# polarsignals/frostdb

Hardware: AMD Instinct MI355X
Metric: rows/sec filter+group-by on 1B-row Prometheus Arrow (HBM-resident); achieved HBM GB/s vs peak (higher is better)
Workload: dtype f64; 1 GPU; headline: Prometheus schema, labels.code=='200' + SUM(value) GROUP BY labels.path; total_rows=1000000000, rows_per_gpu=1000000000, records_per_gpu=40, groups=1025, parallelism=1 GPU

## Files before the change

### frostdb_amd/csrc/fdb_capi.cpp

```cpp
#include <cstring>
#include <new>
#include <string>
#include <vector>

#include "fdb_codec.h"
#include "fdb_comm.h"
#include "fdb_context.h"
#include "fdb_dynamic.h"
#include "fdb_jit.h"
#include "fdb_mergepath.h"
#include "fdb_mergerec.h"
#include "fdb_plan.h"
#include "fdb_pqwrite_host.h"
#include "fdb_record.h"
#include "fdb_regex.h"
#include "fdb_sort.h"
#include "fdb_sortkey.h"
#include "fdb_take.h"

struct fdb_plan {
  std::unique_ptr<fdb::DynamicAggs> dyn;
  fdb_plan_desc main_desc;
  fdb::Plan plan;
  fdb_plan(const fdb_plan_desc* d, int dev)
// ... 106 lines not shown
      fdb::widen_indices_mapped(src, width + 10, table, width == -12 ? 4 : 16, dst, (size_t)n);
      return;
    }
    fdb::widen_indices(src, width, dst, (size_t)n);
  });
}

int fdb_selftest_scan_cache(const uint32_t* indices, int64_t rows, int32_t width, int device, uint8_t* out, int64_t out_bytes) {
  return guard(nullptr, [&] {
    if (indices == nullptr || out == nullptr || rows <= 0 || rows > ((int64_t)1 << 28) || (width != 1 && width != 2) || out_bytes != (rows * width + 15) / 16 * 16)
      throw fdb::Error(FDB_ERR_INVALID, "scan cache: 1 to 2^28 rows, width 1 or 2, out_bytes = rows * width rounded up to 16");
    fdb::CallScope call(device);
    void* d_src = call.alloc(fdb::values_slot((size_t)rows, 4));
    void* d_dst = call.alloc(fdb::values_slot((size_t)rows, (size_t)width));
    fdb::hip_check(hipMemcpyAsync(d_src, indices, (size_t)rows * 4, hipMemcpyHostToDevice, call.ctx->stream), "scan cache: copy in");
    fdb::hip_check(fdb_launch_narrow_indices((const uint32_t*)d_src, d_dst, rows, width, call.ctx->stream), "scan cache: builder");
    fdb::hip_check(hipMemcpyAsync(out, d_dst, (size_t)out_bytes, hipMemcpyDeviceToHost, call.ctx->stream), "scan cache: copy out");
    fdb::hip_check(hipStreamSynchronize(call.ctx->stream), "scan cache: wait");
    for (int64_t i = 0; i < rows; i++) {
      const int64_t at = fdb::scan_cache_position(i, rows, width);
      const uint32_t got = width == 1 ? out[at] : (uint32_t)out[2 * at] | ((uint32_t)out[2 * at + 1] << 8);
      if (got != (indices[i] & (width == 1 ? 0xFFu : 0xFFFFu))) throw fdb::Error(FDB_ERR_INVALID, "scan cache: row " + std::to_string(i) + " is not at its position");
    }
  });
}

int fdb_selftest_exact_sum(const double* x, int64_t n, double* out) {
  return guard(nullptr, [&] {
    if (n < 0 || out == nullptr || (n > 0 && x == nullptr)) throw fdb::Error(FDB_ERR_INVALID, "exact sum: n >= 0 and non-null buffers");
    long long limbs[FDB_EXACT_LIMBS] = {0};
    unsigned long long flags = 0;
    int64_t since = 0;
    for (int64_t i = 0; i < n; i++) {
      unsigned long long bits;
      std::memcpy(&bits, x + i, 8);
      int k; long long d0, d1, d2;
      const unsigned long long f = fdb_exact_split(bits, &k, &d0, &d1, &d2);
      if (f != 0ull) { flags |= f; continue; }
      limbs[k] += d0; limbs[k + 1] += d1; limbs[k + 2] += d2;
      if (++since == ((int64_t)1 << 30)) { fdb_exact_normalize(limbs); since = 0; }
    }
    const unsigned long long r = fdb_exact_round(limbs, flags);
    std::memcpy(out, &r, 8);
  });
}

// ... 845 lines not shown
```

### frostdb_amd/csrc/fdb_dense.cpp

```cpp
#include "fdb_plan.h"
#include "fdb_jit.h"

#include "fdb_context.h"
#include "fdb_launch_plan.h"
#include "fdb_plan_internal.h"

#include <optional>

namespace fdb {

struct Plan::DenseLaunch {
  Plan& P;
  const DeviceBatch* const* bs;
  std::vector<Resolved>& Rs;
  std::vector<std::vector<int>>& part_gcols;
  const std::vector<int>& live;
  const bool fixed_order;
  PhaseTimer& pt;
  const bool jit_possible;
  const int sub;
  FdbScanArgs& args(int i) { return Rs[(size_t)i].args; }

  std::optional<StageScope> stage_scope;
  LutClasses luts;
  size_t lut_lds_max = 0;

  bool slots_ok = false;
  bool interp_ok = true;
  int two_phase = 0;

  LdsPlan lds;
  FoldFuncs funcs;

  struct Narrowed { int part, k, col; bool late; const void* wide; int64_t saved; };
  std::vector<Narrowed> narrowed;

  hipFunction_t jit_fn = nullptr;
  std::string shape_key;
  int jit_block = 0;
  bool slot_kernel = false;
  int per_cu = 1;
  int tile_rows = 0;

  DenseLaunch(Plan& p, const DeviceBatch* const* b, std::vector<Resolved>& rs, std::vector<std::vector<int>>& gc, const std::vector<int>& lv, bool fixed, PhaseTimer& t)
      : P(p), bs(b), Rs(rs), part_gcols(gc), live(lv), fixed_order(fixed), pt(t), jit_possible(p.jit_possible()), sub(p.sub_tiles == 4 ? 0 : p.sub_tiles) {}

  void bind_group_columns();
  void stage_luts();
  void assign_all_slots();
  void plan_lds();
  bool specialisable() const { return slots_ok && P.sub_tiles != 4 && lds.lds_bytes <= 150 * 1024; }
  void narrow_slots();
  void narrow_pool(bool late);
  void widen_slots();
  bool choose_kernel();
  bool split_by_shape();
  void launch();
  void launch_slots();
  void launch_sequential();
  unsigned long long* alloc_partials(int grid);
  void fold_partials(unsigned long long* partials, int grid);
};

void Plan::DenseLaunch::bind_group_columns() {
  for (int i : live) {
    Resolved& R = Rs[(size_t)i];
    FdbScanArgs& a = R.args;
    for (const GroupRes& gr : R.groups) {
      FdbGroupCol& G = a.gcols[a.n_gcols];
      const DevColumn& c = bs[i]->cols[(size_t)gr.ci];
      G.idx = (const uint32_t*)c.d_values;
      G.validity = c.d_validity;
      G.lut_len = (uint32_t)gr.lut->size();
      G.lut_lds = FDB_NO_LDS;
      G.slot = -1;
      R.gcol_col[a.n_gcols] = gr.ci;
      const size_t off = R.blob.add(gr.lut->data(), gr.lut->size() * 4);
      R.luts.push_back(PendingLut{1, a.n_gcols, off, gr.lut->size() * 4});
      part_gcols[(size_t)i].push_back(gr.gi);
      a.n_gcols++;
    }
  }
  std::vector<uint32_t> caps;
  for (const GroupColState& g : P.gcols_) caps.push_back((uint32_t)g.values.size() + 1);
  P.ensure_layout(caps);
  pt.mark("layout");
}

void Plan::DenseLaunch::stage_luts() {
  for (int i : live) luts.add(Rs[(size_t)i]);
  stage_scope.emplace(P.ctx_);
  unsigned char* d_blob = luts.blob.bytes.empty() ? nullptr : (unsigned char*)P.upload(luts.blob.bytes.data(), luts.blob.bytes.size());
  size_t k = 0;
  for (int i : live) lut_lds_max = std::max(lut_lds_max, luts.place(k++, d_blob, Rs[(size_t)i]));
}

void Plan::DenseLaunch::assign_all_slots() {
  slots_ok = P.rows_per_thread == 0;
  std::vector<int> layouts;
  for (int i : live) {
    Resolved& R = Rs[(size_t)i];
// ... 18 lines not shown
    size_t k = 0;
    for (int i : live)
      if (layouts[k++] == 1 && assign_slots(*bs[i], Rs[(size_t)i], 2, jit_possible) != 2) throw Error(FDB_ERR_INVALID, "internal: slot re-assignment failed");
  }
}

void Plan::DenseLaunch::plan_lds() {
  const size_t acc_bytes = align_up((size_t)P.n_slots_ * 4, 16) + (size_t)P.n_slots_ * 8 * P.aggs_.size();
  lds = fdb::plan_lds(lut_lds_max, acc_bytes, P.aggs_.size(), jit_possible, slots_ok, fixed_order, P.use_partials, P.grid_override,
                      P.grid_override > 0 ? P.grid_override : fdb_scan_default_grid(P.device_));
  if (!lds.refusal.empty()) throw Error(FDB_ERR_UNSUPPORTED, lds.refusal);
  int32_t func[FDB_MAX_AGGS], type[FDB_MAX_AGGS];
  for (size_t j = 0; j < P.aggs_.size(); j++) { func[j] = args(live[0]).aggs[j].func; type[j] = P.aggs_[j].type; }
  funcs = fold_funcs(func, type, P.aggs_.size());
  for (int i : live) { args(i).lds_lut_bytes = (uint32_t)lut_lds_max; args(i).lds_acc = lds.lds_acc; args(i).cache_slots = lds.cache_slots; }
  pt.mark("lut upload");
}

void Plan::DenseLaunch::narrow_slots() {
  if (!specialisable() || !jit_possible) return;
  narrow_pool(false);
  if (two_phase) narrow_pool(true);
}
void Plan::DenseLaunch::narrow_pool(bool late) {
  const FdbScanArgs& a0 = args(live[0]);
  const int n4 = late ? a0.n_l4 : a0.n_c4;
  for (int i : live) if ((late ? args(i).n_l4 : args(i).n_c4) != n4) return;
  for (int k = 0; k < n4; k++) {
    int w = 0;
    for (int i : live) {
      const Resolved& R = Rs[(size_t)i];
      const int ci = late ? R.l4_col[k] : R.c4_col[k];
      const int wi = (late ? R.args.l4[k] : R.args.c4[k]).values == nullptr || ci < 0 ? 4 : scan_cache_width(*bs[i], (size_t)ci);
      w = w == 0 || w == wi ? wi : 4;
      if (w == 4) break;
    }
    if (w >= 4) continue;
    for (int i : live) {
      Resolved& R = Rs[(size_t)i];
      const int ci = late ? R.l4_col[k] : R.c4_col[k];
      FdbColSlot& sl = late ? R.args.l4[k] : R.args.c4[k];
      bool counted = false;
      for (const Narrowed& nw : narrowed) if (nw.part == i && nw.col == ci) counted = true;
      const int64_t saved = counted ? 0 : bs[i]->rows * (int64_t)(4 - w);
      narrowed.push_back(Narrowed{i, k, ci, late, sl.values, saved});
      sl.values = scan_cache_get(*bs[i], (size_t)ci, P.stream_);
      (late ? R.args.wl4 : R.args.w4)[k] = (uint8_t)w;
      R.bytes -= saved;
    }
  }
}
void Plan::DenseLaunch::widen_slots() {
  for (const Narrowed& nw : narrowed) {
    Resolved& R = Rs[(size_t)nw.part];
    (nw.late ? R.args.l4 : R.args.c4)[nw.k].values = nw.wide;
    (nw.late ? R.args.wl4 : R.args.w4)[nw.k] = 0;
    R.bytes += nw.saved;
  }
  narrowed.clear();
}

bool Plan::DenseLaunch::choose_kernel() {
  jit_block = fixed_order ? 256 : sub == 1 ? 512 : sub == 2 ? 256 : sub == 3 ? 1024 : 0;
  if (specialisable()) {
    JitShape shape;
    bool same = true, first = true;
    const FdbScanArgs& args0 = args(live[0]);
    for (int i : live) {
      if (first) { shape = jit_shape(args0, two_phase != 0, jit_block ? jit_block : 256); first = false; }
      else if (!jit_shape_merge_args(&shape, args0, args(i), two_phase != 0)) { same = false; break; }
    }
    if (!same && live.size() > 1 && jit_possible && split_by_shape()) return false;
    {
      int regs_per_slot = 2;
      for (const AggState& A : P.aggs_) if (A.func != FDB_AGG_COUNT || P.final_stage_) regs_per_slot += 2;
      if (P.n_slots_ >= 1 && P.n_slots_ <= 8 && (int)P.n_slots_ * regs_per_slot <= 48) shape.reg_slots = (int)P.n_slots_;
    }
    shape.wave_tables = fixed_order;
// ... 55 lines not shown
  parts.reserve(live.size());
  for (int i : live) parts.push_back(args(i));
  const int64_t total_tiles = assign_tiles(parts.data(), parts.size(), tile_rows);
  if (grid > total_tiles) grid = (int)total_tiles;
  unsigned long long* partials = alloc_partials(grid);
  for (FdbScanArgs& a : parts) a.partials = partials;
  bool fill_rides = false;
  if (P.state_virgin_ && jit_fn != nullptr && partials != nullptr && (uint64_t)P.slots_alloc_ * (1 + P.aggs_.size()) < (1ull << 32)) {
    FdbScanArgs& a0 = parts[0];
    a0.fill_state = P.d_state_;
    a0.fill_words = (uint32_t)(P.slots_alloc_ * (1 + P.aggs_.size()));
    a0.fill_alloc = (uint32_t)P.slots_alloc_;
    P.state_idents(a0.fill_idents);
    fill_rides = true;
  } else {
    P.materialize_state();
  }
  P.trace("before scan");
  pt.mark("parts build");
  const FdbScanArgs* d_parts = (const FdbScanArgs*)P.upload(parts.data(), parts.size() * sizeof(FdbScanArgs));
  P.ctx_->flush_staging();
  pt.mark("parts upload");
  P.trace("after upload");
  if (pt.on)
    print_dense_launch(jit_fn != nullptr ? "fdb_plan_kernel" : "scan_slots_kernel", shape_key, parts.data(), parts.size(), total_tiles, grid, jit_fn != nullptr ? jit_block : 0, lds.lds_bytes,
                       two_phase, lds.lds_acc, lds.cache_slots, lut_lds_max, per_cu, tile_rows, fill_rides, partials != nullptr);
  P.timed([&] {
    if (jit_fn != nullptr) hip_check(jit_launch(jit_fn, d_parts, (int)parts.size(), total_tiles, parts[0], grid, jit_block, lds.lds_bytes, P.stream_), "scan launch");
    else hip_check(fdb_launch_scan_slots(d_parts, (int)parts.size(), parts[0], total_tiles, grid, lds.lds_bytes, two_phase, sub, P.stream_), "scan launch");
  });
  if (fill_rides) P.state_virgin_ = false;
  P.last_kernel_ = jit_fn != nullptr ? "fdb_plan_kernel" : "scan_slots_kernel";
  pt.mark("scan launch");
  P.trace("after scan");
  fold_partials(partials, grid);
  P.trace("after reduce");
  P.stat_launches += 1;
}

void Plan::DenseLaunch::launch_sequential() {
  const int rpt = P.rows_per_thread == 8 ? 8 : 4;
  P.materialize_state();
  P.ctx_->flush_staging();
  for (int i : live) {
    FdbScanArgs& a = args(i);
    if (a.n_expr > 0) throw Error(FDB_ERR_UNSUPPORTED, "computed (projected) columns are not supported by the sequential kernel (too many referenced columns)");
    a.n_c4 = a.n_c8 = 0;
    const int grid = fdb_scan_grid(a, lds.base_grid, rpt);
    a.partials = alloc_partials(grid);
// ... 24 lines not shown
```

### frostdb_amd/csrc/fdb_kernels.h

```cpp
#pragma once

#ifndef FDB_DEVICE_ONLY
#include <hip/hip_runtime_api.h>
#include <stdint.h>
#else
typedef signed char int8_t; typedef unsigned char uint8_t; typedef short int16_t; typedef unsigned short uint16_t;
typedef int int32_t; typedef unsigned int uint32_t; typedef long int64_t; typedef unsigned long uint64_t;
#endif

#define FDB_MAX_LEAVES 12
#define FDB_MAX_CODE 32
#define FDB_MAX_DENSE_GCOLS 8
#define FDB_MAX_HASH_GCOLS 64
#define FDB_MAX_AGGS 8
#define FDB_MAX_C4 4
#define FDB_MAX_C8 2
#define FDB_MAX_L4 2
#define FDB_MAX_L8 3
#define FDB_ARG_C4 6
#define FDB_ARG_C8 4
#define FDB_ARG_L4 6
#define FDB_ARG_L8 4
#define FDB_BLOCK 1024
#define FDB_LDS_BUDGET 65536
// ... 482 lines not shown
  uint32_t epoch;
  uint32_t stage_off;
  uint32_t status_off;
  uint32_t place_off;
  const unsigned long long* zero;
  int32_t n_zero;
};

#define FDB_PROJECT_MAX_OUT 16
#define FDB_PROJECT_TILE 1024
struct FdbProjectOut {
  void* values;
  uint8_t* validity;
};
struct FdbProjectPart { FdbProjectOut out[FDB_PROJECT_MAX_OUT]; };

#ifndef FDB_DEVICE_ONLY
hipError_t fdb_launch_scan_dense(const FdbScanArgs& args, int grid_blocks, size_t lds_bytes, int rows_per_thread,
                                 hipStream_t stream);
int fdb_scan_grid(const FdbScanArgs& args, int grid_blocks, int rows_per_thread);
hipError_t fdb_launch_reduce_partials(const unsigned long long* partials, int n_blocks, int n_arrays, uint32_t n_slots,
                                      unsigned long long* state, uint64_t state_stride, const int32_t* funcs, unsigned long long* host_out, hipStream_t stream);
hipError_t fdb_launch_narrow_indices(const uint32_t* src, void* dst, int64_t rows, int width, hipStream_t stream);
hipError_t fdb_launch_stream_read(const void* src, int64_t bytes, unsigned long long* out, hipStream_t stream);
hipError_t fdb_launch_scan_slots(const FdbScanArgs* d_parts, int n_parts, const FdbScanArgs& common, int64_t total_tiles, int grid_blocks,
                                 size_t lds_bytes, int two_phase, int mode, hipStream_t stream);
int fdb_slot_geometry(int two_phase, int mode, int lds_acc, size_t lds_bytes, int device, int* tile_rows, int* blocks_per_cu);
hipError_t fdb_launch_ordered_to_f64(unsigned long long* v, int64_t n, hipStream_t stream);
hipError_t fdb_launch_fill_state(unsigned long long* base, int64_t n, int n_arrays, const unsigned long long* idents, hipStream_t stream);
hipError_t fdb_launch_state_to_host(const unsigned long long* state, unsigned long long* host_out, uint32_t n_slots, uint64_t stride, int n_arrays, hipStream_t stream);
hipError_t fdb_launch_state_pack(const unsigned long long* state, unsigned long long* packed, uint32_t n_slots, uint64_t stride, int n_arrays, hipStream_t stream);
hipError_t fdb_launch_state_fold_ranks(const unsigned long long* gathered, int n_ranks, uint32_t n_slots, int n_arrays, const int32_t* ops, unsigned long long* state,
                                       uint64_t stride, unsigned long long* host_out, hipStream_t stream);
hipError_t fdb_launch_merge_u64(unsigned long long* dst, const unsigned long long* src, const uint32_t* map,
                                int64_t n, int32_t func, int32_t is_f64, hipStream_t stream, const unsigned long long* src_cnt = nullptr);
#define FDB_COMPACT_BLOCK 256
#define FDB_COMPACT_SUB 8
#define FDB_COMPACT_SUBTILE (64 * 4)
#define FDB_COMPACT_TILE (FDB_COMPACT_SUBTILE * FDB_COMPACT_SUB)
#define FDB_COMPACT_STREAM_WAVE_LDS 6144
#define FDB_COMPACT_WAVE_LDS 5120
hipError_t fdb_launch_filter_flags(const FdbScanArgs& args, uint8_t* masks, uint32_t* tile_counts, int device, hipStream_t stream);
hipError_t fdb_launch_compact_col(int width, const void* src, const uint8_t* src_valid, void* dst, uint8_t* dst_valid, const uint8_t* masks,
                                  const uint32_t* tile_offsets, int64_t n_rows, unsigned long long* null_count, int device, hipStream_t stream);
struct FdbCompactRec { int64_t tile_begin; int64_t n_rows; };
struct FdbCompactCol { const void* src; const uint8_t* src_valid; void* dst; uint8_t* dst_valid; int32_t width; int32_t nullable; };
// ... 63 lines not shown
```

### frostdb_amd/csrc/fdb_kernels.hip

```cpp
#include <hip/hip_runtime.h>

#define FDB_DEVICE_HELPERS 1
#include <cstdlib>
#include <cstring>

#include "fdb_kernels.h"
#include "fdb_record.h"

namespace {

constexpr int OP_EQ = 1, OP_NOT_EQ = 2, OP_LT = 3, OP_LT_EQ = 4, OP_GT = 5, OP_GT_EQ = 6;
constexpr int AGG_SUM = 1, AGG_MIN = 2, AGG_MAX = 3, AGG_COUNT = 4;

__device__ __forceinline__ long long f64_to_ordered(double d) {
  long long b = __double_as_longlong(d);
  return b ^ ((b >> 63) & 0x7FFFFFFFFFFFFFFFLL);
}
__device__ __forceinline__ long long f64_minmax_key(double d, bool is_min) {
  d += 0.0;
  const long long k = f64_to_ordered(d);
  return d != d ? (is_min ? FDB_I64_MAX : FDB_I64_MIN) : k;
}

typedef uint32_t u32x4 __attribute__((ext_vector_type(4)));
// ... 2014 lines not shown
      hipLaunchKernelGGL((scan_dense_kernel<4, true>), grid, block, lds_bytes, stream, args);
    } else {
      hipLaunchKernelGGL((scan_dense_kernel<4, false>), grid, block, lds_bytes, stream, args);
    }
  }
  return hipGetLastError();
}

__global__ __launch_bounds__(256) void stream_read_kernel(const u32x4* __restrict__ src, int64_t n_vec, unsigned long long* out) {
  const int64_t i = (int64_t)blockIdx.x * 256 + threadIdx.x;
  if (i >= n_vec) return;
  const u32x4 v = __builtin_nontemporal_load(as_global(src + i));
  if ((v.x ^ v.y ^ v.z ^ v.w) == 0x9E3779B9u) out[0] = 1;
}

hipError_t fdb_launch_stream_read(const void* src, int64_t bytes, unsigned long long* out, hipStream_t stream) {
  const int64_t n_vec = bytes / 16;
  if (n_vec <= 0) return hipSuccess;
  hipLaunchKernelGGL(stream_read_kernel, dim3((unsigned)((n_vec + 255) / 256)), dim3(256), 0, stream, reinterpret_cast<const u32x4*>(src), n_vec, out);
  return hipGetLastError();
}

namespace {
template <int W>
__global__ __launch_bounds__(256) void narrow_indices_kernel(const u32x4* __restrict__ src, u32x4* __restrict__ dst, int64_t rows, int64_t n_vec) {
  const int64_t i = (int64_t)blockIdx.x * 256 + threadIdx.x;
  if (i >= n_vec) return;
  constexpr int PER = 16 / W;
  constexpr int NV = PER / 4;
  constexpr int64_t VB = fdb::kScanCacheBlock * W / 16;
  const int64_t r0 = i * PER;
  const bool interleaved = r0 + PER <= rows / fdb::kScanCacheBlock * fdb::kScanCacheBlock;
  const int64_t s0 = interleaved ? (i / VB) * (fdb::kScanCacheBlock / 4) + ((i % VB) / 64) * (64 * NV) + (i % 64) : i * NV;
  const int64_t sd = interleaved ? 64 : 1;
  uint32_t w[4] = {0u, 0u, 0u, 0u};
#pragma unroll
  for (int k = 0; k < NV; k++) {
    const u32x4 v = __builtin_nontemporal_load(as_global(src + s0 + k * sd));
    const uint32_t e[4] = {v.x, v.y, v.z, v.w};
#pragma unroll
    for (int q = 0; q < 4; q++) {
      const int r = k * 4 + q;
      const uint32_t x = interleaved || r0 + r < rows ? (e[q] & (W == 1 ? 0xFFu : 0xFFFFu)) : 0u;
      w[(r * W) / 4] |= x << (8 * ((r * W) % 4));
    }
  }
  u32x4 out; out.x = w[0]; out.y = w[1]; out.z = w[2]; out.w = w[3];
  dst[i] = out;
}
}

hipError_t fdb_launch_narrow_indices(const uint32_t* src, void* dst, int64_t rows, int width, hipStream_t stream) {
  if (rows <= 0) return hipSuccess;
  if (width != 1 && width != 2) return hipErrorInvalidValue;
  const int64_t per = 16 / width, n_vec = (rows + per - 1) / per;
  const unsigned grid = (unsigned)((n_vec + 255) / 256);
  if (width == 1) hipLaunchKernelGGL(narrow_indices_kernel<1>, dim3(grid), dim3(256), 0, stream, reinterpret_cast<const u32x4*>(src), reinterpret_cast<u32x4*>(dst), rows, n_vec);
  else hipLaunchKernelGGL(narrow_indices_kernel<2>, dim3(grid), dim3(256), 0, stream, reinterpret_cast<const u32x4*>(src), reinterpret_cast<u32x4*>(dst), rows, n_vec);
  return hipGetLastError();
}

namespace {
__global__ void ordered_to_f64_kernel(unsigned long long* v, int64_t n) {
  for (int64_t i = (int64_t)blockIdx.x * blockDim.x + threadIdx.x; i < n; i += (int64_t)gridDim.x * blockDim.x) {
    const long long k = (long long)v[i];
    v[i] = (unsigned long long)(k ^ ((k >> 63) & 0x7FFFFFFFFFFFFFFFLL));
  }
}
}

hipError_t fdb_launch_ordered_to_f64(unsigned long long* v, int64_t n, hipStream_t stream) {
  if (n <= 0) return hipSuccess;
  int blocks = (int)((n + 255) / 256);
  if (blocks > 4096) blocks = 4096;
  hipLaunchKernelGGL(ordered_to_f64_kernel, dim3(blocks), dim3(256), 0, stream, v, n);
  return hipGetLastError();
}

hipError_t fdb_launch_fill_state(unsigned long long* base, int64_t n, int n_arrays, const unsigned long long* idents, hipStream_t stream) {
  if (n <= 0 || n_arrays <= 0) return hipSuccess;
  FillIdents f;
  for (int a = 0; a < 1 + FDB_MAX_AGGS; a++) f.v[a] = a < n_arrays ? idents[a] : 0ull;
// ... 810 lines not shown
```

### frostdb_amd/csrc/fdb_plan_internal.h

```cpp
#pragma once

#include <algorithm>
#include <chrono>
#include <cstdio>
#include <cstdlib>
#include <cstring>
#include <exception>
#include <functional>
#include <memory>
#include <string>
#include <vector>

#include "fdb_context.h"
#include "fdb_plan.h"

namespace fdb {

bool is_leaf_op(int32_t op);

struct PhaseTimer {
  bool on;
  std::chrono::steady_clock::time_point t;
  PhaseTimer() : on(std::getenv("FDB_PROFILE") != nullptr), t(std::chrono::steady_clock::now()) {}
  void mark(const char* what) {
    if (!on) return;
    auto n = std::chrono::steady_clock::now();
    std::fprintf(stderr, "[fdb] %-20s %8.1f us\n", what, std::chrono::duration<double, std::micro>(n - t).count());
    t = n;
  }
};

inline void print_dense_launch(const char* kernel, const std::string& shape_key, const FdbScanArgs* parts, size_t n_parts, int64_t total_tiles, int grid, int block,
                               size_t lds_bytes, int two_phase, int lds_acc, int cache_slots, size_t lut_lds_max, int per_cu, int tile_rows, bool fill_rides, bool partials) {
  std::string s;
  for (size_t p = 0; p < n_parts; p++) {
    s += " " + std::to_string(parts[p].lut_class) + ":";
    for (int k = 0; k < parts[p].n_c4; k++) s += std::to_string((int)parts[p].w4[k]);
    s += "/";
    for (int k = 0; k < parts[p].n_l4; k++) s += std::to_string((int)parts[p].wl4[k]);
  }
  std::fprintf(stderr, "[fdb] dense launch %s shape=%s parts=%zu total_tiles=%lld grid=%d block=%d lds_bytes=%zu two_phase=%d lds_acc=%d cache_slots=%d lut_lds_max=%zu "
               "per_cu=%d tile_rows=%d fill=%d partials=%d class:w4/wl4=%s\n", kernel, shape_key.empty() ? "-" : shape_key.c_str(), n_parts, (long long)total_tiles, grid, block,
               lds_bytes, two_phase, lds_acc, cache_slots, lut_lds_max, per_cu, tile_rows, (int)fill_rides, (int)partials, s.c_str());
}

struct Blob {
  std::vector<uint8_t> bytes;
  size_t add(const void* p, size_t n) {
    const size_t off = align_up(bytes.size(), 16);
    bytes.resize(off + std::max<size_t>(n, 1), 0);
    if (n) std::memcpy(bytes.data() + off, p, n);
    return off;
  }
};

struct PendingLut { int kind; int index; size_t blob_off; size_t len_bytes; };

inline size_t place_luts(const std::vector<PendingLut>& luts, unsigned char* d_blob, size_t lds_off, FdbScanArgs* a) {
  for (const PendingLut& p : luts) {
    const bool in_lds = p.len_bytes <= 16384 && lds_off + p.len_bytes <= 32768;
    uint32_t lds = FDB_NO_LDS;
    if (in_lds) { lds = (uint32_t)lds_off; lds_off = align_up(lds_off + p.len_bytes, 16); }
// ... 92 lines not shown
```

### frostdb_amd/csrc/fdb_record.cpp

```cpp
#include "fdb_record.h"

#include "fdb_context.h"
#include "fdb_plan.h"

namespace fdb {

CallScope::CallScope(int device) {
  hip_check(hipSetDevice(device), "hipSetDevice");
  ctx = Context::acquire(device);
}

CallScope::~CallScope() {
  (void)hipStreamSynchronize(ctx->stream);
  for (void* p : scratch) ctx->dev_free(p);
  ctx->reset_staging();
  Context::release(ctx);
}

void* CallScope::alloc(size_t bytes) {
  void* p = ctx->dev_alloc(bytes);
  scratch.push_back(p);
  return p;
}

int scan_cache_width(const DeviceBatch& b, size_t c) {
  if (b.arena_ctx != nullptr || b.arena_borrowed || b.rows < kScanCacheMinRows) return 4;
  const DevColumn& col = b.cols[c];
  if (col.kind != ColKind::DICT || col.dict == nullptr || col.d_values == nullptr) return 4;
  return narrow_width(col.dict->values.size());
}

const void* scan_cache_get(const DeviceBatch& b, size_t c, hipStream_t stream) {
  const int width = scan_cache_width(b, c);
  if (width >= 4) throw Error(FDB_ERR_INVALID, "internal: no narrow-index cache for column " + b.cols[c].name);
  std::lock_guard<std::mutex> lk(b.scan_cache_mu);
  ScanCache& sc = b.scan_cache;
  if (sc.cols.empty()) sc.cols.resize(b.cols.size());
  ScanCache::Col& e = sc.cols[c];
  if (e.d != nullptr) return e.d;
  const size_t bytes = values_slot((size_t)b.rows, (size_t)width);
  void* d = device_pool_alloc(b.device, bytes);
  hipError_t err = fdb_launch_narrow_indices((const uint32_t*)b.cols[c].d_values, d, b.rows, width, stream);
  if (err == hipSuccess) err = hipStreamSynchronize(stream);
  if (err != hipSuccess) { device_pool_free(b.device, d); hip_check(err, "narrow-index cache"); }
  e.d = d; e.width = width; e.bytes = bytes;
  sc.bytes += (int64_t)bytes;
  return d;
}

void require_values(const DeviceBatch& in, const char* what) {
  for (const DevColumn& c : in.cols)
    if (c.d_values == nullptr && in.rows > 0)
      throw Error(FDB_ERR_UNSUPPORTED, std::string(what) + ": column type " + c.format + " (" + c.name + ") is not supported on the device path");
}

void finish_column(DeviceBatch* b, size_t c, int64_t nulls, void* values, void* bitmap) {
  b->payload_bytes += finish_column(&b->cols[c], b->rows, nulls, values, bitmap);
}

RecordBuilder::RecordBuilder(int device, int64_t rows) : out_(new DeviceBatch()), rows_(rows) {
  out_->device = device;
  out_->rows = rows;
}

RecordBuilder::RecordBuilder(RecordBuilder&&) noexcept = default;
RecordBuilder::~RecordBuilder() = default;

void RecordBuilder::add(const std::string& name, const std::string& format, ColKind kind, std::shared_ptr<HostDict> dict, bool may_have_nulls) {
// ... 34 lines not shown
```

### frostdb_amd/csrc/fdb_record.h

```cpp
#pragma once

#include <cstddef>
#include <cstdint>
#include <memory>
#include <string>
#include <vector>

#include "fdb_arrow.h"

namespace fdb {

inline size_t align_up(size_t v, size_t a) { return (v + a - 1) / a * a; }
constexpr size_t kTailPad = 256;
constexpr size_t kNoSlot = (size_t)-1;

inline size_t value_width(ColKind kind) { return kind == ColKind::DICT || kind == ColKind::STR ? 4 : 8; }
inline size_t values_slot(size_t rows, size_t width) { return align_up(rows * width + kTailPad, 256); }
inline size_t bitmap_slot(size_t rows) { return align_up((rows + 63) / 64 * 8 + kTailPad, 256); }

#if defined(__HIPCC__)
#define FDB_RECORD_HD __host__ __device__
#else
#define FDB_RECORD_HD
#endif
constexpr int64_t kScanCacheBlock = 1024;
FDB_RECORD_HD inline int64_t scan_cache_position(int64_t i, int64_t rows, int width) {
  if (i >= rows / kScanCacheBlock * kScanCacheBlock) return i;
  const int64_t b = i / kScanCacheBlock, j = i % kScanCacheBlock, u = j / 256, l = (j % 256) / 4, r = j % 4;
  return width == 1 ? kScanCacheBlock * b + 16 * l + 4 * u + r : kScanCacheBlock * b + 512 * (u / 2) + 8 * l + 4 * (u % 2) + r;
}

struct RecordLayout {
  struct Col { size_t val_off, bit_off; };
  std::vector<Col> cols;
  size_t total = 0;
  void add(size_t rows, size_t width, bool bitmap) {
    Col c{total, kNoSlot};
    total += values_slot(rows, width);
    if (bitmap) { c.bit_off = total; total += bitmap_slot(rows); }
    cols.push_back(c);
  }
};

struct DevColumn {
  std::string name;
  std::string format;
  ColKind kind = ColKind::OTHER;
  int64_t length = 0;
  int64_t null_count = 0;
  void* d_values = nullptr;
  uint8_t* d_validity = nullptr;
  std::shared_ptr<HostDict> dict;
// ... 16 lines not shown
#include <exception>

#include <hip/hip_runtime_api.h>

namespace fdb {

class Context;
struct DeviceBatch;

struct DrainOnUnwind {
  hipStream_t s; int n = std::uncaught_exceptions();
  ~DrainOnUnwind() { if (std::uncaught_exceptions() > n) (void)hipStreamSynchronize(s); }
};

struct CallScope {
  Context* ctx = nullptr;
  std::vector<void*> scratch;
  explicit CallScope(int device);
  ~CallScope();
  CallScope(const CallScope&) = delete;
  void* alloc(size_t bytes);
};

constexpr int64_t kScanCacheMinRows = (int64_t)1 << 20;
inline int narrow_width(size_t entries) { return entries <= 256 ? 1 : entries <= 65536 ? 2 : 4; }
struct ScanCache {
  struct Col { void* d = nullptr; int width = 0; size_t bytes = 0; };
  std::vector<Col> cols;
  int64_t bytes = 0;
};
int scan_cache_width(const DeviceBatch& b, size_t c);
const void* scan_cache_get(const DeviceBatch& b, size_t c, hipStream_t stream);

void require_values(const DeviceBatch& in, const char* what);

void finish_column(DeviceBatch* b, size_t c, int64_t nulls, void* values, void* bitmap);

class RecordBuilder {
 public:
  RecordBuilder(int device, int64_t rows);
  RecordBuilder(RecordBuilder&&) noexcept;
  ~RecordBuilder();
  void add(const std::string& name, const std::string& format, ColKind kind, std::shared_ptr<HostDict> dict, bool may_have_nulls);
  void allocate();
  void* values(size_t c) const;
  uint8_t* validity(size_t c) const;
  size_t bitmap_slot_bytes() const { return bitmap_slot((size_t)rows_); }
  std::unique_ptr<DeviceBatch> finish(const unsigned long long* nulls);
  static std::unique_ptr<DeviceBatch> schema_of(const DeviceBatch& in);

 private:
  std::unique_ptr<DeviceBatch> out_;
  RecordLayout layout_;
  int64_t rows_;
// ... 5 lines not shown
```

### frostdb_amd/physicalplan.py

```python
from __future__ import annotations

import ctypes
import os
import threading
from typing import Any, Callable, List, Optional, Sequence

import pyarrow as pa

from .arrow_c import ArrowArray, ArrowSchema, ExportedBatch, import_batch
from .logicalplan import AggregationFunction, Column, Expr, expr_name, to_desc

_HERE = os.path.dirname(os.path.abspath(__file__))
LIB_PATH = os.path.join(_HERE, "libfrostdb_amd.so")

FDB_OK, FDB_ERR_INVALID, FDB_ERR_UNSUPPORTED, FDB_ERR_NOT_FOUND, FDB_ERR_DEVICE, FDB_ERR_OOM, FDB_ERR_STATE = range(7)


class FdbError(RuntimeError):
    def __init__(self, code: int, msg: str):
        super().__init__(f"frostdb_amd error {code}: {msg}")
        self.code = code
        self.msg = msg


# ... 54 lines not shown
    L.fdb_parquet_stats.argtypes = [P(i64), P(ctypes.c_double), P(ctypes.c_double), P(i64), P(i64)]
    L.fdb_jit_stats.argtypes = [P(i64), P(ctypes.c_double), P(i64)]
    L.fdb_plan_merge_ms.argtypes = [vp, P(ctypes.c_double)]
    L.fdb_plan_set_timing.argtypes = [vp, i32]
    L.fdb_plan_stream.argtypes = [vp, P(vp)]
    L.fdb_plan_set_tuning.argtypes = [vp, i32, i32]
    L.fdb_plan_set_deterministic.argtypes = [vp, i32]
    L.fdb_plan_set_exact_sums.argtypes = [vp, i32]
    L.fdb_selftest_exact_sum.argtypes = [vp, i64, vp]
    L.fdb_snappy_decode_pages.argtypes = [vp, i64, vp, i32, vp, i64, ctypes.c_int, vp, P(ctypes.c_double)]
    L.fdb_lz4_decode_pages.argtypes = [vp, i64, vp, i32, vp, i64, ctypes.c_int, vp, P(ctypes.c_double)]
    L.fdb_parquet_device_pages.argtypes = [ctypes.c_int, P(i64), P(i64)]
    L.fdb_plan_state_arrays.argtypes = [vp, P(i32)]
    L.fdb_plan_state_array_op.argtypes = [vp, i32, P(i32)]
    L.fdb_plan_group_schema.argtypes = [vp, vp, vp]
    L.fdb_plan_seed_groups.argtypes = [vp, vp, vp]
    L.fdb_plan_hash_export.argtypes = [vp, vp, i32, ctypes.POINTER(ctypes.c_void_p), ctypes.POINTER(ctypes.c_int64), ctypes.POINTER(i32)]
    L.fdb_plan_hash_import.argtypes = [vp, vp, ctypes.c_int64]
    L.fdb_read_ceiling.argtypes = [ctypes.c_int, ctypes.c_int64, i32, ctypes.POINTER(ctypes.c_double)]
    L.fdb_plan_last_kernel.argtypes = [vp]
    L.fdb_arrow_roundtrip.argtypes = [vp, vp, vp, vp]
    L.fdb_selftest_widen.argtypes = [vp, i32, vp, i64]
    L.fdb_selftest_scan_cache.argtypes = [vp, i64, i32, ctypes.c_int, vp, i64]
    L.fdb_plan_explain.argtypes = [vp, ctypes.c_char_p, i64, P(i64)]
    L.fdb_plan_last_kernel.restype = ctypes.c_char_p
    L.fdb_comm_unique_id.argtypes = [vp]
    L.fdb_comm_init_rank.argtypes = [vp, i32, i32, ctypes.c_int, P(vp)]
    L.fdb_comm_init_all.argtypes = [P(ctypes.c_int), i32, P(vp)]
    L.fdb_comm_init_local.argtypes = [P(ctypes.c_int), i32, P(vp)]
    L.fdb_comm_rank.argtypes = [vp]
    L.fdb_comm_rank.restype = i32
    L.fdb_comm_size.argtypes = [vp]
    L.fdb_comm_size.restype = i32
    L.fdb_plan_push_many.argtypes = [vp, vp, vp, i32, P(i32)]
    L.fdb_plan_push_many.restype = i32
    L.fdb_comm_transport_ranks.argtypes = [vp]
    L.fdb_comm_transport_ranks.restype = i32
    L.fdb_comm_last_error.argtypes = [vp]
    L.fdb_comm_last_error.restype = ctypes.c_char_p
    L.fdb_comm_destroy.argtypes = [vp]
    L.fdb_comm_destroy.restype = None
    L.fdb_plan_allreduce.argtypes = [vp, vp, P(i32)]
    L.fdb_plan_exchange.argtypes = [vp, vp, P(vp)]
    L.fdb_live_allocations.argtypes = [P(i64), P(i64), P(i64)]
    L.fdb_plan_filter_batch.argtypes = [vp, vp, P(vp), P(i64)]
    L.fdb_plan_finish_batch.argtypes = [vp, P(vp), P(i64)]
# ... 1212 lines not shown
```

### include/frostdb_amd.h

```cpp
#ifndef FROSTDB_AMD_H
#define FROSTDB_AMD_H

#include <stdint.h>
#include "arrow_c_data.h"

#ifdef __cplusplus
extern "C" {
#endif

#if defined(__GNUC__) || defined(__clang__)
#define FDB_API __attribute__((visibility("default")))
#else
#define FDB_API
#endif

typedef enum fdb_status {
  FDB_OK = 0,
  FDB_ERR_INVALID = 1,
  FDB_ERR_UNSUPPORTED = 2,
  FDB_ERR_NOT_FOUND = 3,
  FDB_ERR_DEVICE = 4,
  FDB_ERR_OOM = 5,
  FDB_ERR_STATE = 6
} fdb_status;
// ... 97 lines not shown
  int32_t n_groups;
  const fdb_group_expr* groups;
  int32_t final_stage;
  int32_t n_projections;
  const fdb_projection* projections;
  fdb_regex_match_fn regex_match;
  void* regex_user;
  int32_t ordered;
  int32_t _pad2;
} fdb_plan_desc;

typedef struct fdb_plan fdb_plan;
typedef struct fdb_batch fdb_batch;

FDB_API const char* fdb_version(void);
FDB_API const char* fdb_last_error(void);
FDB_API int fdb_device_count(int* n_devices);
FDB_API int fdb_read_ceiling(int device, int64_t bytes, int32_t reps, double* gb_per_s);

FDB_API int fdb_arrow_roundtrip(struct ArrowArray* batch, struct ArrowSchema* schema, struct ArrowArray* out, struct ArrowSchema* out_schema);
FDB_API int fdb_regex_match(const char* pattern, int64_t pattern_len, const uint8_t* value, int64_t value_len, int32_t* matched);
FDB_API int fdb_selftest_widen(const void* src, int32_t width, uint32_t* dst, int64_t n);
FDB_API int fdb_selftest_scan_cache(const uint32_t* indices, int64_t rows, int32_t width, int device, uint8_t* out, int64_t out_bytes);

FDB_API int fdb_plan_create(const fdb_plan_desc* desc, int device, fdb_plan** out);
FDB_API int fdb_plan_push(fdb_plan* plan, struct ArrowArray* batch, struct ArrowSchema* schema);
FDB_API int fdb_plan_push_many(fdb_plan* plan, struct ArrowArray* const* batches, struct ArrowSchema* const* schemas, int32_t n, int32_t* n_pushed);
FDB_API int fdb_plan_push_batch(fdb_plan* plan, const fdb_batch* batch);
FDB_API int fdb_plan_push_batches(fdb_plan* plan, const fdb_batch* const* batches, int32_t n);
FDB_API int fdb_plan_finish(fdb_plan* plan, struct ArrowArray* out, struct ArrowSchema* out_schema, int64_t* n_rows);
FDB_API int fdb_plan_finish_next(fdb_plan* plan, struct ArrowArray* out, struct ArrowSchema* out_schema, int64_t* n_rows, int32_t* emitted);
FDB_API int fdb_plan_merge(fdb_plan* dst, fdb_plan* src);
FDB_API int fdb_plan_filter(fdb_plan* plan, struct ArrowArray* batch, struct ArrowSchema* schema,
                    struct ArrowArray* out, struct ArrowSchema* out_schema, int64_t* n_selected);
FDB_API int fdb_plan_select(fdb_plan* plan, struct ArrowArray* batch, struct ArrowSchema* schema,
                    uint32_t* indices, int64_t capacity, int64_t* n_selected);
FDB_API int fdb_plan_filter_batch(fdb_plan* plan, const fdb_batch* batch, fdb_batch** out, int64_t* n_selected);
FDB_API int fdb_plan_finish_batch(fdb_plan* plan, fdb_batch** out, int64_t* n_rows);
FDB_API int fdb_plan_filter_batches(fdb_plan* plan, const fdb_batch* const* batches, int32_t n, fdb_batch** out, int64_t* n_selected);
FDB_API int fdb_plan_select_batch(fdb_plan* plan, const fdb_batch* batch, uint32_t* dev_indices, int64_t capacity, int64_t* n_selected);

typedef struct fdb_project_col {
  int32_t kind;
  int32_t _pad;
  const char* name;
} fdb_project_col;
// ... 173 lines not shown
```

Baseline: 545.8 billion rows/s.

## Fold null validity into narrowed dictionary-index scan cache as a null entry

When building the narrow (1/2-byte) dictionary-index cache for a nullable column, the builder now writes a reserved null index for invalid rows. The scan then drops that column's validity bitmap read and instead extends the group LUT with a zero null entry. This removes per-row bitmap traffic and bit tests from the hot scan, at the cost of a slightly longer LUT and extra bookkeeping to restore the wide pointers and validity on fallback. It only applies when the column has nulls and the dictionary leaves a spare code; if the benchmark's group/filter columns have no nulls, the path is not used.

```diff
diff --git a/frostdb_amd/csrc/fdb_capi.cpp b/frostdb_amd/csrc/fdb_capi.cpp
--- a/frostdb_amd/csrc/fdb_capi.cpp
+++ b/frostdb_amd/csrc/fdb_capi.cpp
@@ -152,6 +152,23 @@
       const uint32_t got = width == 1 ? out[at] : (uint32_t)out[2 * at] | ((uint32_t)out[2 * at + 1] << 8);
       if (got != (indices[i] & (width == 1 ? 0xFFu : 0xFFFFu))) throw fdb::Error(FDB_ERR_INVALID, "scan cache: row " + std::to_string(i) + " is not at its position");
     }
+  });
+}
+
+int fdb_selftest_scan_cache_nulls(const uint32_t* indices, const uint8_t* validity, int64_t rows, int64_t entries, int32_t width, int device, uint8_t* out, int64_t out_bytes) {
+  return guard(nullptr, [&] {
+    if (indices == nullptr || validity == nullptr || out == nullptr || rows <= 0 || rows > ((int64_t)1 << 28) || (width != 1 && width != 2) ||
+        entries < 0 || entries > (width == 1 ? 255 : 65535) || out_bytes != (rows * width + 15) / 16 * 16)
+      throw fdb::Error(FDB_ERR_INVALID, "scan cache: 1 to 2^28 rows, width 1 or 2, entries <= 255 / 65 535, out_bytes = rows * width rounded up to 16");
+    fdb::CallScope call(device);
+    void* d_src = call.alloc(fdb::values_slot((size_t)rows, 4));
+    uint8_t* d_bits = (uint8_t*)call.alloc(fdb::bitmap_slot((size_t)rows));
+    void* d_dst = call.alloc(fdb::values_slot((size_t)rows, (size_t)width));
+    fdb::hip_check(hipMemcpyAsync(d_src, indices, (size_t)rows * 4, hipMemcpyHostToDevice, call.ctx->stream), "scan cache: copy in");
+    fdb::hip_check(hipMemcpyAsync(d_bits, validity, (size_t)(rows + 7) / 8, hipMemcpyHostToDevice, call.ctx->stream), "scan cache: copy in");
+    fdb::hip_check(fdb_launch_narrow_indices((const uint32_t*)d_src, d_bits, (uint32_t)entries, d_dst, rows, width, call.ctx->stream), "scan cache: builder");
+    fdb::hip_check(hipMemcpyAsync(out, d_dst, (size_t)out_bytes, hipMemcpyDeviceToHost, call.ctx->stream), "scan cache: copy out");
+    fdb::hip_check(hipStreamSynchronize(call.ctx->stream), "scan cache: wait");
   });
 }
 
diff --git a/frostdb_amd/csrc/fdb_dense.cpp b/frostdb_amd/csrc/fdb_dense.cpp
--- a/frostdb_amd/csrc/fdb_dense.cpp
+++ b/frostdb_amd/csrc/fdb_dense.cpp
@@ -32,7 +32,7 @@
   LdsPlan lds;
   FoldFuncs funcs;
 
-  struct Narrowed { int part, k, col; bool late; const void* wide; int64_t saved; };
+  struct Narrowed { int part, k, col; bool late; const void* wide; int64_t saved; const uint8_t* validity; bool folded; };
   std::vector<Narrowed> narrowed;
 
   hipFunction_t jit_fn = nullptr;
@@ -71,12 +71,14 @@
       const DevColumn& c = bs[i]->cols[(size_t)gr.ci];
       G.idx = (const uint32_t*)c.d_values;
       G.validity = c.d_validity;
-      G.lut_len = (uint32_t)gr.lut->size();
+      const size_t null_entry = scan_cache_folded(*bs[i], (size_t)gr.ci) && gr.lut->size() <= c.dict->values.size() ? 1 : 0;
+      G.lut_len = (uint32_t)(gr.lut->size() + null_entry);
       G.lut_lds = FDB_NO_LDS;
       G.slot = -1;
       R.gcol_col[a.n_gcols] = gr.ci;
       const size_t off = R.blob.add(gr.lut->data(), gr.lut->size() * 4);
-      R.luts.push_back(PendingLut{1, a.n_gcols, off, gr.lut->size() * 4});
+      R.blob.bytes.resize(R.blob.bytes.size() + null_entry * 4, 0);
+      R.luts.push_back(PendingLut{1, a.n_gcols, off, (gr.lut->size() + null_entry) * 4});
       part_gcols[(size_t)i].push_back(gr.gi);
       a.n_gcols++;
     }
@@ -141,6 +143,11 @@
   narrow_pool(false);
   if (two_phase) narrow_pool(true);
 }
+static bool validity_leaf_reads(const FdbScanArgs& a, int k) {
+  for (int l = 0; l < a.n_leaves; l++)
+    if (a.leaves[l].kind == FDB_LEAF_VALIDITY && !a.leaves[l].wide && a.leaves[l].slot == k) return true;
+  return false;
+}
 void Plan::DenseLaunch::narrow_pool(bool late) {
   const FdbScanArgs& a0 = args(live[0]);
   const int n4 = late ? a0.n_l4 : a0.n_c4;
@@ -162,8 +169,10 @@
       bool counted = false;
       for (const Narrowed& nw : narrowed) if (nw.part == i && nw.col == ci) counted = true;
       const int64_t saved = counted ? 0 : bs[i]->rows * (int64_t)(4 - w);
-      narrowed.push_back(Narrowed{i, k, ci, late, sl.values, saved});
+      const bool fold = sl.validity != nullptr && scan_cache_folded(*bs[i], (size_t)ci) && !(!late && validity_leaf_reads(R.args, k));
+      narrowed.push_back(Narrowed{i, k, ci, late, sl.values, saved, sl.validity, fold});
       sl.values = scan_cache_get(*bs[i], (size_t)ci, P.stream_);
+      if (fold) sl.validity = nullptr;
       (late ? R.args.wl4 : R.args.w4)[k] = (uint8_t)w;
       R.bytes -= saved;
     }
@@ -173,6 +182,7 @@
   for (const Narrowed& nw : narrowed) {
     Resolved& R = Rs[(size_t)nw.part];
     (nw.late ? R.args.l4 : R.args.c4)[nw.k].values = nw.wide;
+    (nw.late ? R.args.l4 : R.args.c4)[nw.k].validity = nw.validity;
     (nw.late ? R.args.wl4 : R.args.w4)[nw.k] = 0;
     R.bytes += nw.saved;
   }
@@ -274,9 +284,13 @@
   P.ctx_->flush_staging();
   pt.mark("parts upload");
   P.trace("after upload");
-  if (pt.on)
+  if (pt.on) {
+    std::vector<uint32_t> folded(parts.size(), 0u);
+    for (const Narrowed& nw : narrowed)
+      if (nw.folded) folded[(size_t)(std::find(live.begin(), live.end(), nw.part) - live.begin())] |= 1u << ((nw.late ? 16 : 0) + nw.k);
     print_dense_launch(jit_fn != nullptr ? "fdb_plan_kernel" : "scan_slots_kernel", shape_key, parts.data(), parts.size(), total_tiles, grid, jit_fn != nullptr ? jit_block : 0, lds.lds_bytes,
-                       two_phase, lds.lds_acc, lds.cache_slots, lut_lds_max, per_cu, tile_rows, fill_rides, partials != nullptr);
+                       two_phase, lds.lds_acc, lds.cache_slots, lut_lds_max, per_cu, tile_rows, fill_rides, partials != nullptr, folded);
+  }
   P.timed([&] {
     if (jit_fn != nullptr) hip_check(jit_launch(jit_fn, d_parts, (int)parts.size(), total_tiles, parts[0], grid, jit_block, lds.lds_bytes, P.stream_), "scan launch");
     else hip_check(fdb_launch_scan_slots(d_parts, (int)parts.size(), parts[0], total_tiles, grid, lds.lds_bytes, two_phase, sub, P.stream_), "scan launch");
diff --git a/frostdb_amd/csrc/fdb_kernels.h b/frostdb_amd/csrc/fdb_kernels.h
--- a/frostdb_amd/csrc/fdb_kernels.h
+++ b/frostdb_amd/csrc/fdb_kernels.h
@@ -528,6 +528,7 @@
 hipError_t fdb_launch_reduce_partials(const unsigned long long* partials, int n_blocks, int n_arrays, uint32_t n_slots,
                                       unsigned long long* state, uint64_t state_stride, const int32_t* funcs, unsigned long long* host_out, hipStream_t stream);
 hipError_t fdb_launch_narrow_indices(const uint32_t* src, void* dst, int64_t rows, int width, hipStream_t stream);
+hipError_t fdb_launch_narrow_indices(const uint32_t* src, const uint8_t* validity, uint32_t null_index, void* dst, int64_t rows, int width, hipStream_t stream);
 hipError_t fdb_launch_stream_read(const void* src, int64_t bytes, unsigned long long* out, hipStream_t stream);
 hipError_t fdb_launch_scan_slots(const FdbScanArgs* d_parts, int n_parts, const FdbScanArgs& common, int64_t total_tiles, int grid_blocks,
                                  size_t lds_bytes, int two_phase, int mode, hipStream_t stream);
diff --git a/frostdb_amd/csrc/fdb_kernels.hip b/frostdb_amd/csrc/fdb_kernels.hip
--- a/frostdb_amd/csrc/fdb_kernels.hip
+++ b/frostdb_amd/csrc/fdb_kernels.hip
@@ -2060,8 +2060,9 @@
 }
 
 namespace {
-template <int W>
-__global__ __launch_bounds__(256) void narrow_indices_kernel(const u32x4* __restrict__ src, u32x4* __restrict__ dst, int64_t rows, int64_t n_vec) {
+template <int W, bool FOLD>
+__global__ __launch_bounds__(256) void narrow_indices_kernel(const u32x4* __restrict__ src, const uint8_t* __restrict__ validity, uint32_t null_index, u32x4* __restrict__ dst,
+                                                             int64_t rows, int64_t n_vec) {
   const int64_t i = (int64_t)blockIdx.x * 256 + threadIdx.x;
   if (i >= n_vec) return;
   constexpr int PER = 16 / W;
@@ -2072,14 +2073,21 @@
   const int64_t s0 = interleaved ? (i / VB) * (fdb::kScanCacheBlock / 4) + ((i % VB) / 64) * (64 * NV) + (i % 64) : i * NV;
   const int64_t sd = interleaved ? 64 : 1;
   uint32_t w[4] = {0u, 0u, 0u, 0u};
+  u32x4 in[NV];
+  uint32_t valid[NV];
 #pragma unroll
   for (int k = 0; k < NV; k++) {
-    const u32x4 v = __builtin_nontemporal_load(as_global(src + s0 + k * sd));
-    const uint32_t e[4] = {v.x, v.y, v.z, v.w};
+    in[k] = __builtin_nontemporal_load(as_global(src + s0 + k * sd));
+    valid[k] = FOLD ? (uint32_t)validity[(s0 + k * sd) >> 1] >> (4 * (int)((s0 + k * sd) & 1)) : 0xFu;
+  }
+#pragma unroll
+  for (int k = 0; k < NV; k++) {
+    const uint32_t e[4] = {in[k].x, in[k].y, in[k].z, in[k].w};
 #pragma unroll
     for (int q = 0; q < 4; q++) {
       const int r = k * 4 + q;
-      const uint32_t x = interleaved || r0 + r < rows ? (e[q] & (W == 1 ? 0xFFu : 0xFFFFu)) : 0u;
+      const uint32_t idx = (valid[k] >> q) & 1u ? (e[q] & (W == 1 ? 0xFFu : 0xFFFFu)) : null_index;
+      const uint32_t x = interleaved || r0 + r < rows ? idx : 0u;
       w[(r * W) / 4] |= x << (8 * ((r * W) % 4));
     }
   }
@@ -2088,14 +2096,26 @@
 }
 }
 
-hipError_t fdb_launch_narrow_indices(const uint32_t* src, void* dst, int64_t rows, int width, hipStream_t stream) {
+namespace {
+template <bool FOLD>
+hipError_t launch_narrow_indices(const uint32_t* src, const uint8_t* validity, uint32_t null_index, void* dst, int64_t rows, int width, hipStream_t stream) {
   if (rows <= 0) return hipSuccess;
   if (width != 1 && width != 2) return hipErrorInvalidValue;
   const int64_t per = 16 / width, n_vec = (rows + per - 1) / per;
   const unsigned grid = (unsigned)((n_vec + 255) / 256);
-  if (width == 1) hipLaunchKernelGGL(narrow_indices_kernel<1>, dim3(grid), dim3(256), 0, stream, reinterpret_cast<const u32x4*>(src), reinterpret_cast<u32x4*>(dst), rows, n_vec);
-  else hipLaunchKernelGGL(narrow_indices_kernel<2>, dim3(grid), dim3(256), 0, stream, reinterpret_cast<const u32x4*>(src), reinterpret_cast<u32x4*>(dst), rows, n_vec);
-  return hipGetLastError();
+  if (width == 1) hipLaunchKernelGGL((narrow_indices_kernel<1, FOLD>), dim3(grid), dim3(256), 0, stream, reinterpret_cast<const u32x4*>(src), validity, null_index, reinterpret_cast<u32x4*>(dst), rows, n_vec);
+  else hipLaunchKernelGGL((narrow_indices_kernel<2, FOLD>), dim3(grid), dim3(256), 0, stream, reinterpret_cast<const u32x4*>(src), validity, null_index, reinterpret_cast<u32x4*>(dst), rows, n_vec);
+  return hipGetLastError();
+}
+}
+
+hipError_t fdb_launch_narrow_indices(const uint32_t* src, void* dst, int64_t rows, int width, hipStream_t stream) {
+  return launch_narrow_indices<false>(src, nullptr, 0u, dst, rows, width, stream);
+}
+
+hipError_t fdb_launch_narrow_indices(const uint32_t* src, const uint8_t* validity, uint32_t null_index, void* dst, int64_t rows, int width, hipStream_t stream) {
+  if (validity == nullptr || null_index > (width == 1 ? 0xFFu : 0xFFFFu)) return hipErrorInvalidValue;
+  return launch_narrow_indices<true>(src, validity, null_index, dst, rows, width, stream);
 }
 
 namespace {
diff --git a/frostdb_amd/csrc/fdb_plan_internal.h b/frostdb_amd/csrc/fdb_plan_internal.h
--- a/frostdb_amd/csrc/fdb_plan_internal.h
+++ b/frostdb_amd/csrc/fdb_plan_internal.h
@@ -31,13 +31,15 @@
 };
 
 inline void print_dense_launch(const char* kernel, const std::string& shape_key, const FdbScanArgs* parts, size_t n_parts, int64_t total_tiles, int grid, int block,
-                               size_t lds_bytes, int two_phase, int lds_acc, int cache_slots, size_t lut_lds_max, int per_cu, int tile_rows, bool fill_rides, bool partials) {
+                               size_t lds_bytes, int two_phase, int lds_acc, int cache_slots, size_t lut_lds_max, int per_cu, int tile_rows, bool fill_rides, bool partials,
+                               const std::vector<uint32_t>& folded = std::vector<uint32_t>()) {
   std::string s;
   for (size_t p = 0; p < n_parts; p++) {
     s += " " + std::to_string(parts[p].lut_class) + ":";
-    for (int k = 0; k < parts[p].n_c4; k++) s += std::to_string((int)parts[p].w4[k]);
+    const uint32_t f = p < folded.size() ? folded[p] : 0u;
+    for (int k = 0; k < parts[p].n_c4; k++) s += std::to_string((int)parts[p].w4[k]) + ((f >> k) & 1u ? "n" : "");
     s += "/";
-    for (int k = 0; k < parts[p].n_l4; k++) s += std::to_string((int)parts[p].wl4[k]);
+    for (int k = 0; k < parts[p].n_l4; k++) s += std::to_string((int)parts[p].wl4[k]) + ((f >> (16 + k)) & 1u ? "n" : "");
   }
   std::fprintf(stderr, "[fdb] dense launch %s shape=%s parts=%zu total_tiles=%lld grid=%d block=%d lds_bytes=%zu two_phase=%d lds_acc=%d cache_slots=%d lut_lds_max=%zu "
                "per_cu=%d tile_rows=%d fill=%d partials=%d class:w4/wl4=%s\n", kernel, shape_key.empty() ? "-" : shape_key.c_str(), n_parts, (long long)total_tiles, grid, block,
diff --git a/frostdb_amd/csrc/fdb_record.cpp b/frostdb_amd/csrc/fdb_record.cpp
--- a/frostdb_amd/csrc/fdb_record.cpp
+++ b/frostdb_amd/csrc/fdb_record.cpp
@@ -30,6 +30,12 @@
   return narrow_width(col.dict->values.size());
 }
 
+bool scan_cache_folded(const DeviceBatch& b, size_t c) {
+  if (scan_cache_width(b, c) >= 4) return false;
+  const DevColumn& col = b.cols[c];
+  return col.d_validity != nullptr && scan_cache_folds(col.dict->values.size(), col.null_count, b.rows);
+}
+
 const void* scan_cache_get(const DeviceBatch& b, size_t c, hipStream_t stream) {
   const int width = scan_cache_width(b, c);
   if (width >= 4) throw Error(FDB_ERR_INVALID, "internal: no narrow-index cache for column " + b.cols[c].name);
@@ -40,10 +46,12 @@
   if (e.d != nullptr) return e.d;
   const size_t bytes = values_slot((size_t)b.rows, (size_t)width);
   void* d = device_pool_alloc(b.device, bytes);
-  hipError_t err = fdb_launch_narrow_indices((const uint32_t*)b.cols[c].d_values, d, b.rows, width, stream);
+  const bool folded = scan_cache_folded(b, c);
+  hipError_t err = folded ? fdb_launch_narrow_indices((const uint32_t*)b.cols[c].d_values, b.cols[c].d_validity, (uint32_t)b.cols[c].dict->values.size(), d, b.rows, width, stream)
+                          : fdb_launch_narrow_indices((const uint32_t*)b.cols[c].d_values, d, b.rows, width, stream);
   if (err == hipSuccess) err = hipStreamSynchronize(stream);
   if (err != hipSuccess) { device_pool_free(b.device, d); hip_check(err, "narrow-index cache"); }
-  e.d = d; e.width = width; e.bytes = bytes;
+  e.d = d; e.width = width; e.bytes = bytes; e.folded = folded;
   sc.bytes += (int64_t)bytes;
   return d;
 }
diff --git a/frostdb_amd/csrc/fdb_record.h b/frostdb_amd/csrc/fdb_record.h
--- a/frostdb_amd/csrc/fdb_record.h
+++ b/frostdb_amd/csrc/fdb_record.h
@@ -28,6 +28,14 @@
   if (i >= rows / kScanCacheBlock * kScanCacheBlock) return i;
   const int64_t b = i / kScanCacheBlock, j = i % kScanCacheBlock, u = j / 256, l = (j % 256) / 4, r = j % 4;
   return width == 1 ? kScanCacheBlock * b + 16 * l + 4 * u + r : kScanCacheBlock * b + 512 * (u / 2) + 8 * l + 4 * (u % 2) + r;
+}
+
+constexpr int64_t kScanCacheMinRows = (int64_t)1 << 20;
+inline int narrow_width(size_t entries) { return entries <= 256 ? 1 : entries <= 65536 ? 2 : 4; }
+inline int scan_cache_width_of(size_t entries, int64_t rows) { return rows < kScanCacheMinRows ? 4 : narrow_width(entries); }
+inline bool scan_cache_folds(size_t entries, int64_t nulls, int64_t rows) {
+  const int w = scan_cache_width_of(entries, rows);
+  return nulls > 0 && w < 4 && entries < ((size_t)1 << (8 * w));
 }
 
 struct RecordLayout {
@@ -90,14 +98,13 @@
   void* alloc(size_t bytes);
 };
 
-constexpr int64_t kScanCacheMinRows = (int64_t)1 << 20;
-inline int narrow_width(size_t entries) { return entries <= 256 ? 1 : entries <= 65536 ? 2 : 4; }
 struct ScanCache {
-  struct Col { void* d = nullptr; int width = 0; size_t bytes = 0; };
+  struct Col { void* d = nullptr; int width = 0; size_t bytes = 0; bool folded = false; };
   std::vector<Col> cols;
   int64_t bytes = 0;
 };
 int scan_cache_width(const DeviceBatch& b, size_t c);
+bool scan_cache_folded(const DeviceBatch& b, size_t c);
 const void* scan_cache_get(const DeviceBatch& b, size_t c, hipStream_t stream);
 
 void require_values(const DeviceBatch& in, const char* what);
diff --git a/frostdb_amd/physicalplan.py b/frostdb_amd/physicalplan.py
--- a/frostdb_amd/physicalplan.py
+++ b/frostdb_amd/physicalplan.py
@@ -100,6 +100,7 @@
     L.fdb_arrow_roundtrip.argtypes = [vp, vp, vp, vp]
     L.fdb_selftest_widen.argtypes = [vp, i32, vp, i64]
     L.fdb_selftest_scan_cache.argtypes = [vp, i64, i32, ctypes.c_int, vp, i64]
+    L.fdb_selftest_scan_cache_nulls.argtypes = [vp, vp, i64, i64, i32, ctypes.c_int, vp, i64]
     L.fdb_plan_explain.argtypes = [vp, ctypes.c_char_p, i64, P(i64)]
     L.fdb_plan_last_kernel.restype = ctypes.c_char_p
     L.fdb_comm_unique_id.argtypes = [vp]
diff --git a/include/frostdb_amd.h b/include/frostdb_amd.h
--- a/include/frostdb_amd.h
+++ b/include/frostdb_amd.h
@@ -143,6 +143,8 @@
 FDB_API int fdb_regex_match(const char* pattern, int64_t pattern_len, const uint8_t* value, int64_t value_len, int32_t* matched);
 FDB_API int fdb_selftest_widen(const void* src, int32_t width, uint32_t* dst, int64_t n);
 FDB_API int fdb_selftest_scan_cache(const uint32_t* indices, int64_t rows, int32_t width, int device, uint8_t* out, int64_t out_bytes);
+FDB_API int fdb_selftest_scan_cache_nulls(const uint32_t* indices, const uint8_t* validity, int64_t rows, int64_t entries, int32_t width, int device, uint8_t* out,
+                                          int64_t out_bytes);
 
 FDB_API int fdb_plan_create(const fdb_plan_desc* desc, int device, fdb_plan** out);
 FDB_API int fdb_plan_push(fdb_plan* plan, struct ArrowArray* batch, struct ArrowSchema* schema);
```

Result: faster. 555.6 billion rows/s, median of 6 (+1.8%).
